# Hcyand/recommender_system

Measured on AMD Instinct MI355X. Metric: CTR forward samples/sec @ batch 4096, 26 sparse×1e7 vocab, dim 16; %HBM roofline, higher is better.
Workload: dtype f32

## Files before the change

### recommender_system_amd/csrc/capi.cpp

```cpp
#include <stdarg.h>
#include <stdio.h>

#include "rs_common.hpp"

namespace rs {
static thread_local char g_err[512] = "";

void set_error(const char* fmt, ...) {
  va_list ap;
  va_start(ap, fmt);
  vsnprintf(g_err, sizeof(g_err), fmt, ap);
  va_end(ap);
}

int launch_status(const char* what) {
  hipError_t e = hipGetLastError();
  if (e != hipSuccess) {
    set_error("%s: HIP launch failed: %s", what, hipGetErrorString(e));
    return RS_ERR_HIP;
  }
  return RS_OK;
}

static thread_local int g_opt[RS_OPT_COUNT] = {0, 1, 0, 0, 0, 0};
static const int g_opt_hi[RS_OPT_COUNT] = {5, 1, 3, 1, 1, 1};
int opt(int option) { return (option >= 0 && option < RS_OPT_COUNT) ? g_opt[option] : 0; }
}

extern "C" int rs_set_option(int option, int value) {
  if (option < 0 || option >= RS_OPT_COUNT || value < 0 || value > rs::g_opt_hi[option]) {
    rs::set_error("rs_set_option: unknown option %d or value %d out of range", option, value);
    return -1;
  }
  const int prev = rs::g_opt[option];
  rs::g_opt[option] = value;
  return prev;
}

extern "C" int rs_get_option(int option) {
  return (option >= 0 && option < RS_OPT_COUNT) ? rs::g_opt[option] : -1;
}

extern "C" const char* rs_version(void) { return "recommender_system_amd 0.1.0 (gfx950)"; }
extern "C" const char* rs_last_error_string(void) { return rs::g_err; }
```

### recommender_system_amd/csrc/deepfm.hip

```cpp
#include <stdlib.h>

#include <type_traits>

#include "embed_fm_body.hpp"
#include "rs_common.hpp"

namespace rs {

template <int KV, int KIND>
__global__ __launch_bounds__(16 * 64) void deepfm_fused(EmbedFmArgs a, MlpArgs t) {
  embed_fm_body<KV, 1, 16, KIND, true, 1>(a, &t, blockIdx.x);
}
template <int KV, int KIND>
__global__ __launch_bounds__(16 * 64) void deepfm_fused_ka(EmbedFmArgs a, MlpArgs t, FieldMeta m) {
  embed_fm_body<KV, 1, 16, KIND, true, 1, false, true>(a, &t, blockIdx.x, &m);
}

constexpr int WS_NL = 8;

__device__ __forceinline__ void lds_wait_ge(int* p, int v, int* err) {
  for (int spins = 0; __hip_atomic_load(p, __ATOMIC_ACQUIRE, __HIP_MEMORY_SCOPE_WORKGROUP) < v; ++spins) {
    if (spins > (1 << 22)) {
      if ((threadIdx.x & 63) == 0) flag_error(err, RS_FLAG_TIMEOUT);
      break;
    }
    __builtin_amdgcn_s_sleep(1);
  }
}
__device__ __forceinline__ void lds_signal(int* p) {
  if ((threadIdx.x & 63) == 0) __hip_atomic_fetch_add(p, 1, __ATOMIC_RELEASE, __HIP_MEMORY_SCOPE_WORKGROUP);
}

template <int KIND, int G, int GWA = 0, int GWB = 0>
__global__ __launch_bounds__(16 * 64) void deepfm_ws(EmbedFmArgs a, MlpArgs t, FieldMeta m) {
  typedef Ids<KIND> I;
  constexpr int NW = 16, F = G - 1, MF = (F + WS_NL - 1) / WS_NL;
  static_assert(F <= 32 && MF <= 4, "deepfm_ws: <= 32 fields");
  extern __shared__ float tsm[];
  __shared__ floatx4 lf_acc[WS_NL][64];
  __shared__ floatx4 lf_q[WS_NL][4];
  __shared__ float fmlog[16];
  __shared__ int cnt[4];
  const int lane = threadIdx.x & 63;
  const int w = __builtin_amdgcn_readfirstlane(threadIdx.x >> 6);
  const int s = lane & 15, kk = lane >> 4;
  const int64_t bt = (int64_t)blockIdx.x * 16 + s;
  const bool valid = bt < a.batch;
  const int64_t b = valid ? bt : a.batch - 1;
  const int RS = t.rs;
  float* par = tsm + 32 * RS + NW * 256;
  floatx4 ring[MLP_R];
  {
    const MlpArgs& a = t;
    MLP_STAMP(0);
  }
  if (threadIdx.x < 4) cnt[threadIdx.x] = 0;
  if (w < WS_NL) {
    const int l = w;
    const float w0v = a.w0[0];
    const int dw = l - (WS_NL - a.DB);
    const bool has_dense = dw >= 0;
    float dx = 0.f, drec = 0.f, dn = 0.f;
    if (has_dense) {
      const int e = 4 * dw + kk;
      dx = a.dense[b * a.dense_stride + (e < a.nd ? e : 0)];
      const float* rec = a.prep + (int64_t)dw * a.dense_rec;
      drec = rec[lane];
      dn = rec[64 + kk];
    }
    typename I::raw_t rid[MF];
    floatx4 bw[MF];
#pragma unroll
    for (int p = 0; p < MF; ++p) {
      const int c = l + WS_NL * p;
      bw[p] = floatx4{0.f, 0.f, 0.f, 0.f};
      if (c < F) {
        rid[p] = I::load(a.ids, b * a.id_stride + c);
        if (s <= a.kfm) bw[p] = *reinterpret_cast<const floatx4*>(a.prep + a.field_base + (int64_t)c * a.field_rec + lane * 4);
      }
    }
    floatx4 xs0[2];
    bool ok0[2];
#pragma unroll
    for (int q = 0; q < 2; ++q) {
      const int c = l + WS_NL * q;
      ok0[q] = false;
      if (q < MF && c < F) {
        int64_t id;
        ok0[q] = I::decode(rid[q], m.voc[c], id);
        xs0[q] = __builtin_nontemporal_load(reinterpret_cast<const floatx4*>(a.table + (m.off[c] + id) * 16) + kk);
      }
    }
    __syncthreads();
    floatx4 ac[4];
#pragma unroll
    for (int c = 0; c < 4; ++c) ac[c] = floatx4{0.f, 0.f, 0.f, 0.f};
    float qn = 0.f;
    if (has_dense) {
      const int e = 4 * dw + kk;
      const float x = e < a.nd ? dx : 0.f;
      ac[0] = mfma16x16x4(x, drec, ac[0]);
      qn = fmaf(x * x, dn, qn);
      tsm[s * RS + F * 16 + e] = x;
      lds_signal(&cnt[0]);
    }
    float nrm[MF][4];
#pragma unroll
    for (int p = 0; p < MF; ++p)
#pragma unroll
      for (int tp = 0; tp < 4; ++tp) nrm[p][tp] = row16_sum(s < a.kfm ? bw[p][tp] * bw[p][tp] : 0.f);
    bool bad = false;
#pragma unroll
    for (int burst = 0; burst < 2; ++burst) {
      floatx4 xs[2];
      bool ok[2];
#pragma unroll
      for (int q = 0; q < 2; ++q) {
        const int p = 2 * burst + q, c = l + WS_NL * p;
        if (burst == 0) {
          xs[q] = xs0[q];
          ok[q] = ok0[q];
          continue;
        }
        ok[q] = false;
        if (p < MF && c < F) {
          int64_t id;
          ok[q] = I::decode(rid[p], m.voc[c], id);
          xs[q] = __builtin_nontemporal_load(reinterpret_cast<const floatx4*>(a.table + (m.off[c] + id) * 16) + kk);
        }
      }
#pragma unroll
      for (int q = 0; q < 2; ++q) {
        const int p = 2 * burst + q, c = l + WS_NL * p;
        if (p < MF && c < F) {
          bad |= !ok[q];
          const floatx4 x = ok[q] ? xs[q] : floatx4{0.f, 0.f, 0.f, 0.f};
          *reinterpret_cast<floatx4*>(tsm + s * RS + c * 16 + 4 * kk) = x;
#pragma unroll
          for (int tp = 0; tp < 4; ++tp) {
            ac[tp] = mfma16x16x4(x[tp], bw[p][tp], ac[tp]);
            qn = fmaf(x[tp] * x[tp], nrm[p][tp], qn);
          }
        }
      }
#ifdef RS_DIAG_STAMPS
      if (!(burst == 1 && (a.ablate & 32)))
#endif
      lds_signal(&cnt[1 + burst]);
      {
        const MlpArgs& a = t;
        MLP_STAMP(2 + burst);
      }
    }
    if (__any(bad && valid) && lane == 0) flag_error(a.err);
    floatx4 acc;
#pragma unroll
    for (int i = 0; i < 4; ++i) acc[i] = (ac[0][i] + ac[1][i]) + (ac[2][i] + ac[3][i]);
    lf_acc[l][lane] = acc;
    qn += __shfl_xor(qn, 16);
    qn += __shfl_xor(qn, 32);
    if (lane < 16) reinterpret_cast<float*>(&lf_q[l][0])[lane] = qn;
    int old = 0;
    if (lane == 0) old = __hip_atomic_fetch_add(&cnt[3], 1, __ATOMIC_ACQ_REL, __HIP_MEMORY_SCOPE_WORKGROUP);
    old = __builtin_amdgcn_readfirstlane(old);
    if (old == WS_NL - 1) {
      floatx4 v = {0.f, 0.f, 0.f, 0.f};
#pragma unroll
      for (int ww = 0; ww < WS_NL; ++ww) {
        const floatx4 pv = lf_acc[ww][lane];
#pragma unroll
        for (int i = 0; i < 4; ++i) v[i] += pv[i];
      }
      const floatx4 q4 = lf_q[s < WS_NL ? s : 0][kk];
#pragma unroll
      for (int i = 0; i < 4; ++i) {
        float tt = s < a.kfm ? v[i] * v[i] : 0.f;
        if (s < WS_NL) tt -= q4[i];
        float ll = s == a.kfm ? v[i] : 0.f;
        tt = row16_sum(tt);
        ll = row16_sum(ll);
        const float fm = (ll + w0v) + 0.5f * tt;
        const int64_t bb = (int64_t)blockIdx.x * 16 + 4 * kk + i;
        if (s == 0) {
          fmlog[4 * kk + i] = fm;
          if (bb < a.batch && a.logit) a.logit[bb] = fm;
        }
      }
    }
  } else {
    const int c8 = w - WS_NL;
    const floatx4* W0 = reinterpret_cast<const floatx4*>(t.prep + t.off[0]) + lane + (int64_t)c8 * G * 64;
    const floatx4* W1 = W0 + (int64_t)WS_NL * G * 64;
    auto grp = [](int i) { return i == 0 ? G - 1 : i - 1; };
    floatx4 r0[3], r1[3];
#pragma unroll
    for (int u = 0; u < 3; ++u) {
      r0[u] = W0[(int64_t)grp(u) * 64];
      r1[u] = W1[(int64_t)grp(u) * 64];
    }
    __syncthreads();
    for (int i = threadIdx.x - WS_NL * 64; i < t.ptot; i += (NW - WS_NL) * 64) par[i] = t.prep[t.wtot + i];
    const int ecol0 = 16 * c8 + s, ecol1 = ecol0 + 16 * WS_NL;
    const float* pb = t.prep + t.wtot + t.poff[0];
    const float eb0 = pb[ecol0], eb1 = pb[ecol1], ea0 = pb[t.Np[0] + ecol0], ea1 = pb[t.Np[0] + ecol1];
    const float* ap = tsm + s * RS + 4 * kk;
    floatx4 acc0 = {0.f, 0.f, 0.f, 0.f}, acc1 = acc0, acc0b = acc0, acc1b = acc0;
    lds_wait_ge(&cnt[0], a.DB, a.err);
    auto step = [&](int i, auto U) {
      constexpr int u = decltype(U)::value;
      const floatx4 av = *reinterpret_cast<const floatx4*>(ap + 16 * grp(i));
      __builtin_amdgcn_sched_barrier(0);
#pragma unroll
      for (int j = 0; j < 4; j += 2) {
        acc0 = mfma16x16x4(av[j], r0[u][j], acc0);
        acc1 = mfma16x16x4(av[j], r1[u][j], acc1);
        acc0b = mfma16x16x4(av[j + 1], r0[u][j + 1], acc0b);
        acc1b = mfma16x16x4(av[j + 1], r1[u][j + 1], acc1b);
      }
      const int nx = i + 3 < G ? i + 3 : G - 1;
      r0[u] = W0[(int64_t)grp(nx) * 64];
      r1[u] = W1[(int64_t)grp(nx) * 64];
      __builtin_amdgcn_sched_barrier(0);
    };
    using U0 = std::integral_constant<int, 0>;
    using U1 = std::integral_constant<int, 1>;
    using U2 = std::integral_constant<int, 2>;
    auto wait_burst = [&](int which) {
      lds_wait_ge(&cnt[1 + which], WS_NL, a.err);
      const MlpArgs& a = t;
      MLP_STAMP(2 + which);
    };
    constexpr int B1 = 1 + 2 * WS_NL;
    if (t.unroll) {
#pragma unroll
      for (int i = 0; i < G; ++i) {
        if (i == 1) wait_burst(0);
        if (i == B1) wait_burst(1);
        if (i % 3 == 0) step(i, U0{});
        else if (i % 3 == 1) step(i, U1{});
        else step(i, U2{});
      }
    } else {
      static_assert((B1 - 2) % 3 == 0 && (G - 1 - B1) % 3 == 0, "deepfm_ws: group / ring phase");
      step(0, U0{});
      wait_burst(0);
      int i = 1;
#pragma unroll 1
      for (; i + 2 < B1; i += 3) {
        step(i, U1{});
        step(i + 1, U2{});
        step(i + 2, U0{});
      }
      step(i, U1{});
      wait_burst(1);
#pragma unroll 1
      for (i = B1; i + 2 < G; i += 3) {
        step(i, U2{});
        step(i + 1, U0{});
        step(i + 2, U1{});
      }
      step(i, U2{});
    }
#pragma unroll
    for (int i = 0; i < 4; ++i) {
      acc0[i] += acc0b[i];
      acc1[i] += acc1b[i];
    }
    float* out = tsm + 16 * RS;
    with_act(t.act[0], [&](auto A) {
#pragma unroll
      for (int r = 0; r < 4; ++r) {
        const int row = 4 * kk + r;
        out[row * RS + ecol0] = mlp_act_c<decltype(A)::value>(acc0[r] + eb0, ea0);
        out[row * RS + ecol1] = mlp_act_c<decltype(A)::value>(acc1[r] + eb1, ea1);
      }
    });
  }
  {
    const MlpArgs& a = t;
    MLP_STAMP(1);
  }
  if constexpr (GWA > 0) {
    if constexpr (GWA == 8 && GWB == 2) {
      mlp_tail_run<NW>(t, tsm, (int64_t)blockIdx.x * 16, fmlog);
    } else {
      floatx4 wr[GWA];
      mlp_tail_fetch<GWA>(t, 1, wr);
      mlp_tail_splitk<NW, GWA, GWB>(t, tsm, (int64_t)blockIdx.x * 16, wr, fmlog, 1);
    }
  } else {
    {
      const int T1 = t.Np[1] >> 4, G1 = t.Kp[1] >> 4;
      const int S1 = mlp_slices(T1, G1, NW);
      if (w < T1 * S1) {
        const MlpItem it = mlp_item(w, T1, G1, S1);
        mlp_ring_fill(ring, reinterpret_cast<const floatx4*>(t.prep + t.off[1]) + lane + (int64_t)it.t * G1 * 64,
                      it.g0, it.g1);
      }
    }
    mlp_tower_tile<NW>(t, tsm, (int64_t)blockIdx.x * 16, ring, fmlog, 1);
  }
}

template <int KIND, int G, int RD, int GWA = 0, int GWB = 0>
__global__ __launch_bounds__(16 * 64) void deepfm_all(EmbedFmArgs a, MlpArgs t, FieldMeta m) {
  typedef Ids<KIND> I;
  constexpr int NW = 16, F = G - 1;
  static_assert(F > 16 && F <= 32, "deepfm_all: 17..32 fields (two per wave at most)");
  static_assert(RD == 3 || RD == 4, "deepfm_all: weight ring 3 or 4 k-groups deep");
  extern __shared__ float tsm[];
  __shared__ floatx4 fm_acc[NW][64];
  __shared__ float fm_q[NW][16];
  __shared__ float fmlog[16];
  const int lane = threadIdx.x & 63;
  const int w = __builtin_amdgcn_readfirstlane(threadIdx.x >> 6);
  const int s = lane & 15, kk = lane >> 4;
  const int64_t bt = (int64_t)blockIdx.x * 16 + s;
  const bool valid = bt < a.batch;
  const int64_t b = valid ? bt : a.batch - 1;
  const int RS = t.rs;
  float* par = tsm + 32 * RS + NW * 256;
  {
    const MlpArgs& a = t;
    MLP_STAMP(0);
  }
  const int c0 = w, c1 = w + 16 < F ? w + 16 : w;
  const bool two = w + 16 < F;
  const typename I::raw_t rid0 = I::load(a.ids, b * a.id_stride + c0);
  const typename I::raw_t rid1 = I::load(a.ids, b * a.id_stride + c1);
  const int dw = w - (NW - 4);
  const bool has_dense = dw >= 0 && dw < a.DB;
  const int dwc = dw < 0 ? 0 : (dw < a.DB ? dw : 0);
  const int de = 4 * dwc + kk;
  const float dxv = a.dense[b * a.dense_stride + (de < a.nd ? de : 0)];
  int64_t id0, id1;
  const bool ok0 = I::decode(rid0, m.voc[c0], id0);
  const bool ok1 = I::decode(rid1, m.voc[c1], id1);
  const floatx4 x0 = __builtin_nontemporal_load(reinterpret_cast<const floatx4*>(a.table + (m.off[c0] + id0) * 16) + kk);
  const floatx4* x1p = reinterpret_cast<const floatx4*>(a.table + (m.off[c1] + id1) * 16) + kk;
  const floatx4* W0 = reinterpret_cast<const floatx4*>(t.prep + t.off[0]) + lane + (int64_t)w * G * 64;
  auto grp = [](int i) { return i == 0 ? G - 1 : i - 1; };
  floatx4 ring[RD];
#pragma unroll
  for (int u = 0; u < RD; ++u) ring[u] = W0[(int64_t)grp(u) * 64];
  const float* drec = a.prep + (int64_t)dwc * a.dense_rec;
  const float drv = drec[lane], dnv = drec[64 + kk];
  const floatx4 bw0 = *reinterpret_cast<const floatx4*>(a.prep + a.field_base + (int64_t)c0 * a.field_rec + lane * 4);
  const floatx4 bw1 = *reinterpret_cast<const floatx4*>(a.prep + a.field_base + (int64_t)c1 * a.field_rec + lane * 4);
  const float w0v = a.w0[0];
  const int npar = t.ptot;
  const int pi = threadIdx.x < npar ? threadIdx.x : 0;
  const float pv = t.prep[t.wtot + pi];
  bool bad = !ok0 || (two && !ok1);
  MacAcc<4> L0;
  const float* ap = tsm + s * RS + 4 * kk;
  floatx4 an = {0.f, 0.f, 0.f, 0.f};
  auto seg_start = [&](int i) { an = *reinterpret_cast<const floatx4*>(ap + 16 * grp(i)); };
  auto step = [&](int i, auto U) {
    constexpr int u = decltype(U)::value;
    const floatx4 av = an;
    if (i != 16 && i + 1 < G) an = *reinterpret_cast<const floatx4*>(ap + 16 * grp(i + 1));
    __builtin_amdgcn_sched_barrier(0);
    L0.mac4(av, ring[u]);
    if (i + RD < G) ring[u] = W0[(int64_t)grp(i + RD) * 64];
    __builtin_amdgcn_sched_barrier(0);
  };
  auto step_i = [&](int i) {
    switch (i % RD) {
      case 0: step(i, std::integral_constant<int, 0>{}); break;
      case 1: step(i, std::integral_constant<int, 1>{}); break;
      case 2: step(i, std::integral_constant<int, 2>{}); break;
      default: step(i, std::integral_constant<int, (RD > 3 ? 3 : 0)>{}); break;
    }
  };
  floatx4 fa = {0.f, 0.f, 0.f, 0.f};
  float qn = 0.f;
  if (dw >= 0) {
    const int e = 4 * dw + kk;
    const float x = e < a.nd ? dxv : 0.f;
    tsm[s * RS + F * 16 + e] = x;
    if (has_dense) {
      fa = mfma16x16x4(x, drv, fa);
      qn = fmaf(x * x, dnv, qn);
    }
  }
  float n0[4], n1[4];
#pragma unroll
  for (int tp = 0; tp < 4; ++tp) {
    n0[tp] = row16_sum(s < a.kfm ? bw0[tp] * bw0[tp] : 0.f);
    n1[tp] = row16_sum(s < a.kfm ? bw1[tp] * bw1[tp] : 0.f);
  }
  if (threadIdx.x < npar) par[pi] = pv;
  auto put_row = [&](int c, const floatx4& xr, bool ok, const floatx4& bw, const float (&nr)[4]) {
    const floatx4 x = ok ? xr : floatx4{0.f, 0.f, 0.f, 0.f};
    *reinterpret_cast<floatx4*>(tsm + s * RS + c * 16 + 4 * kk) = x;
#pragma unroll
    for (int tp = 0; tp < 4; ++tp) {
      fa = mfma16x16x4(x[tp], bw[tp], fa);
      qn = fmaf(x[tp] * x[tp], nr[tp], qn);
    }
  };
  put_row(c0, x0, ok0, bw0, n0);
  __syncthreads();
  {
    const MlpArgs& a = t;
    MLP_STAMP(2);
  }
  const floatx4 x1 = __builtin_nontemporal_load(x1p);
  __builtin_amdgcn_sched_barrier(0);
  seg_start(0);
#pragma unroll
  for (int i = 0; i <= 16; ++i) {
    step_i(i);
    if (i == 8) {
      if (two) put_row(c1, x1, ok1, bw1, n1);
      fm_acc[w][lane] = fa;
      qn += __shfl_xor(qn, 16);
      qn += __shfl_xor(qn, 32);
      if (lane < 16) fm_q[w][lane] = qn;
      if (__any(bad && valid) && lane == 0) flag_error(a.err);
    }
  }
  __syncthreads();
  {
    const MlpArgs& a = t;
    MLP_STAMP(3);
  }
  float fmv[NW];
  {
    const int ln = (w >> 2) * 16 + s, r = w & 3;
#pragma unroll
    for (int ww = 0; ww < NW; ++ww) fmv[ww] = fm_acc[ww][ln][r];
  }
  const float fq = fm_q[s][w];
  seg_start(17);
#pragma unroll
  for (int i = 17; i < G; ++i) step_i(i);
  const floatx4 acc0 = L0.sum();
  constexpr bool TAIL = GWA > 0;
  floatx4 wr[TAIL ? GWA : 1];
  floatx4 tring[MLP_R];
  if constexpr (TAIL) {
    mlp_tail_fetch<GWA>(t, 1, wr);
  } else {
    const int T1 = t.Np[1] >> 4, G1 = t.Kp[1] >> 4;
    const int S1 = mlp_slices(T1, G1, NW);
    if (w < T1 * S1) {
      const MlpItem it = mlp_item(w, T1, G1, S1);
      mlp_ring_fill(tring, reinterpret_cast<const floatx4*>(t.prep + t.off[1]) + lane + (int64_t)it.t * G1 * 64,
                    it.g0, it.g1);
    }
  }
  {
    float* out = tsm + 16 * RS;
    const int col = 16 * w + s;
    const float bc = par[t.poff[0] + col], ac = par[t.poff[0] + t.Np[0] + col];
    with_act(t.act[0], [&](auto A) {
#pragma unroll
      for (int r = 0; r < 4; ++r) out[(4 * kk + r) * RS + col] = mlp_act_c<decltype(A)::value>(acc0[r] + bc, ac);
    });
  }
  {
    float v = 0.f;
#pragma unroll
    for (int ww = 0; ww < NW; ++ww) v += fmv[ww];
    float tq = (s < a.kfm ? v * v : 0.f) - fq;
    float lin = s == a.kfm ? v : 0.f;
    tq = row16_sum(tq);
    lin = row16_sum(lin);
    const float fm = (lin + w0v) + 0.5f * tq;
    if (lane == 0) {
      fmlog[w] = fm;
      const int64_t bb = (int64_t)blockIdx.x * 16 + w;
      if (bb < a.batch && a.logit) a.logit[bb] = fm;
    }
  }
  {
    const MlpArgs& a = t;
    MLP_STAMP(1);
  }
  if constexpr (TAIL) {
    if constexpr (GWA == 8 && GWB == 2) mlp_tail_dispatch<NW>(t, tsm, (int64_t)blockIdx.x * 16, wr, fmlog, 1);
    else mlp_tail_splitk<NW, GWA, GWB>(t, tsm, (int64_t)blockIdx.x * 16, wr, fmlog, 1);
  }
  else mlp_tower_tile<NW>(t, tsm, (int64_t)blockIdx.x * 16, tring, fmlog, 1);
}

static bool deepfm_geom(int nd, int n_fields, int k, int kfm, int n_layers, const int* dims, FmGeom& fg,
                        MlpGeom& mg) {
  if (nd < 0 || n_fields < 1 || n_fields > 128 || kfm < 1 || (k != 8 && k != 16)) return false;
  fg = fm_geom(nd, n_fields, k, kfm);
  if (!fg.mfma || fg.NT != 1) return false;
  if (!mlp_geom(n_layers, dims, mg)) return false;
  return dims[0] == nd + n_fields * k && dims[n_layers] == 1 && mg.lds <= 120 * 1024;
}

static bool deepfm_ws_ok(const EmbedFmArgs& a, const MlpArgs& t, const FieldMeta* hm, int KV) {
  return hm && KV == 4 && a.F == 26 && a.nd >= 13 && a.nd <= 16 && a.DB == 4 && t.L >= 2 &&
         t.Np[0] == 256 && t.Kp[0] == 16 * (a.F + 1) && (t.Np[1] >> 4) >= WS_NL &&
         opt(RS_OPT_DEEPFM_KERNEL) == 0;
}

static bool deepfm_all_ok(const EmbedFmArgs& a, const MlpArgs& t, const FieldMeta* hm, int KV) {
  return hm && KV == 4 && a.F == 26 && a.nd >= 1 && a.nd <= 16 && a.DB <= 4 && t.L >= 2 && t.Np[0] == 256 &&
         t.Kp[0] == 16 * (a.F + 1) && t.ptot <= 1024 && opt(RS_OPT_DEEPFM_KERNEL) >= 2;
}

template <int KV, int KIND>
static void launch_deepfm(const EmbedFmArgs& a, const MlpArgs& t, size_t lds, hipStream_t st,
                          const FieldMeta* hm) {
  const unsigned grid = (unsigned)((a.batch + 15) / 16);
  if constexpr (KV == 4) {
    if (deepfm_all_ok(a, t, hm, KV)) {
      int gwa = 0, gwb = 0;
      const bool tail = mlp_tail_ok(t.Np, t.Kp, t.N, t.L, 1, gwa, gwb) && gwa == 8 && gwb == 2;
      const bool ring4 = opt(RS_OPT_DEEPFM_KERNEL) == 3;
      if (tail && ring4) launch_lds<deepfm_all<KIND, 27, 4, 8, 2>>(grid, 16 * 64, lds, st, a, t, *hm);
      else if (tail) launch_lds<deepfm_all<KIND, 27, 3, 8, 2>>(grid, 16 * 64, lds, st, a, t, *hm);
      else launch_lds<deepfm_all<KIND, 27, 3>>(grid, 16 * 64, lds, st, a, t, *hm);
      return;
    }
    if (deepfm_ws_ok(a, t, hm, KV)) {
      int gwa = 0, gwb = 0;
      if (mlp_tail_ok(t.Np, t.Kp, t.N, t.L, 1, gwa, gwb) && gwa == 8 && gwb == 2)
        launch_lds<deepfm_ws<KIND, 27, 8, 2>>(grid, 16 * 64, lds, st, a, t, *hm);
      else launch_lds<deepfm_ws<KIND, 27>>(grid, 16 * 64, lds, st, a, t, *hm);
      return;
    }
  }
  if (hm && a.F <= 32 && a.DB <= 16) launch_lds<deepfm_fused_ka<KV, KIND>>(grid, 16 * 64, lds, st, a, t, *hm);
  else launch_lds<deepfm_fused<KV, KIND>>(grid, 16 * 64, lds, st, a, t);
}

}

using namespace rs;

extern "C" int rs_deepfm_fused_ok(int nd, int n_fields, int k, int kfm, int n_layers, const int* dims) {
  FmGeom fg;
  MlpGeom mg;
  return dims && deepfm_geom(nd, n_fields, k, kfm, n_layers, dims, fg, mg) ? 1 : 0;
}

static int deepfm_run(const void* ids, int id_kind, int64_t id_stride, const float* dense, int64_t dense_stride,
                      int nd, const float* table, const int64_t* field_offsets, const int64_t* field_vocab,
                      int n_fields, int k, const float* fm_prepared, const float* w0, int kfm, int n_layers,
                      const int* dims, const int* acts, const float* mlp_prepared, float c0, float c1, float* out,
                      float* fm_logit, int64_t batch, int* err_flag, rs_stream_t stream, const FieldMeta* hm) {
  if (batch == 0) return RS_OK;
  FmGeom fg;
  MlpGeom mg;
  RS_REQUIRE(dims && acts, "rs_deepfm_fwd: null dims/acts");
  RS_REQUIRE(deepfm_geom(nd, n_fields, k, kfm, n_layers, dims, fg, mg),
             "rs_deepfm_fwd: unsupported shape (see rs_deepfm_fused_ok)");
  RS_REQUIRE(batch >= 0 && ids && table && field_offsets && field_vocab && fm_prepared && w0 && mlp_prepared && out,
             "rs_deepfm_fwd: null pointer");
  RS_REQUIRE(nd == 0 || dense, "rs_deepfm_fwd: dense is null");
  RS_REQUIRE(id_kind >= RS_ID_I32 && id_kind <= RS_ID_F32, "rs_deepfm_fwd: bad id_kind");
  RS_REQUIRE((uintptr_t)table % 16 == 0, "rs_deepfm_fwd: table must be 16-B aligned");
  MlpArgs t{};
  RS_REQUIRE(mlp_fill_args(mg, acts, mlp_prepared, t), "rs_deepfm_fwd: bad activation");
  t.y = out;
  t.ys = 1;
  t.head = 1;
  t.c0 = c0;
  t.c1 = c1;
  t.M = batch;
  t.dbg = mlp_diag_dbg();
  EmbedFmArgs a = fm_args(ids, id_stride, dense, dense_stride, nd, table, field_offsets, field_vocab, n_fields, k,
                          fm_prepared, w0, kfm, fm_logit, nullptr, batch, err_flag);
  set_geom(a, fg);
#ifdef RS_DIAG_STAMPS
  a.ablate = getenv("RS_ABLATE") ? atoi(getenv("RS_ABLATE")) : 0;
#endif
  hipStream_t st = as_stream(stream);
  with_id_kind(id_kind, [&](auto K) {
    constexpr int KIND = decltype(K)::value;
    if (fg.KV == 2) launch_deepfm<2, KIND>(a, t, mg.lds, st, hm);
    else launch_deepfm<4, KIND>(a, t, mg.lds, st, hm);
  });
  return launch_status("rs_deepfm_fwd");
}

extern "C" int rs_deepfm_fwd(const void* ids, int id_kind, int64_t id_stride, const float* dense,
                             int64_t dense_stride, int nd, const float* table, const int64_t* field_offsets,
                             const int64_t* field_vocab, int n_fields, int k, const float* fm_prepared,
                             const float* w0, int kfm, int n_layers, const int* dims, const int* acts,
                             const float* mlp_prepared, float c0, float c1, float* out, float* fm_logit,
                             int64_t batch, int* err_flag, rs_stream_t stream) {
  return deepfm_run(ids, id_kind, id_stride, dense, dense_stride, nd, table, field_offsets, field_vocab, n_fields, k,
                    fm_prepared, w0, kfm, n_layers, dims, acts, mlp_prepared, c0, c1, out, fm_logit, batch, err_flag,
                    stream, nullptr);
}

extern "C" int rs_deepfm_fwd_hm(const void* ids, int id_kind, int64_t id_stride, const float* dense,
                                int64_t dense_stride, int nd, const float* table, const int64_t* field_offsets,
                                const int64_t* field_vocab, const int64_t* field_offsets_host,
                                const int64_t* field_vocab_host, int n_fields, int k, const float* fm_prepared,
                                const float* w0, int kfm, int n_layers, const int* dims, const int* acts,
                                const float* mlp_prepared, float c0, float c1, float* out, float* fm_logit,
                                int64_t batch, int* err_flag, rs_stream_t stream) {
  RS_REQUIRE(batch == 0 || (field_offsets_host && field_vocab_host), "rs_deepfm_fwd_hm: host metadata missing");
  const bool use = n_fields <= 32 && batch > 0;
  const FieldMeta m = field_meta(field_offsets_host, field_vocab_host, use ? n_fields : 0);
  return deepfm_run(ids, id_kind, id_stride, dense, dense_stride, nd, table, field_offsets, field_vocab, n_fields, k,
                    fm_prepared, w0, kfm, n_layers, dims, acts, mlp_prepared, c0, c1, out, fm_logit, batch, err_flag,
                    stream, use ? &m : nullptr);
}
```

### recommender_system_amd/csrc/embed_fm.hip

```cpp
#include <stdlib.h>

#include <type_traits>

#include "embed_fm_body.hpp"
#include "rs_common.hpp"

namespace rs {

__device__ __forceinline__ float fm_bval(const float* w1, const float* v, int d, int kfm, int e, int colg) {
  if (e >= d) return 0.f;
  if (colg < kfm) return v[(int64_t)e * kfm + colg];
  if (colg == kfm) return w1[e];
  return 0.f;
}

__device__ __forceinline__ float fm_rownorm(const float* v, int d, int kfm, int e) {
  if (e >= d) return 0.f;
  float n = 0.f;
  for (int f = 0; f < kfm; ++f) {
    const float t = v[(int64_t)e * kfm + f];
    n = fmaf(t, t, n);
  }
  return n;
}

__global__ void fm_prepare_mfma(const float* __restrict__ w1, const float* __restrict__ v, int nd, int F,
                                int k, int kfm, int KV, int NT, int DB, int64_t dense_rec,
                                int64_t field_rec, int64_t field_base, int64_t size,
                                float* __restrict__ out) {
  const int d = nd + F * k;
  for (int64_t idx = (int64_t)blockIdx.x * blockDim.x + threadIdx.x; idx < size;
       idx += (int64_t)gridDim.x * blockDim.x) {
    float val;
    if (idx < field_base) {
      const int t = (int)(idx / dense_rec);
      const int r = (int)(idx % dense_rec);
      if (r < NT * 64) {
        const int nt = r / 64, lane = r % 64;
        const int e = 4 * t + (lane >> 4);
        val = (e < nd) ? fm_bval(w1, v, d, kfm, e, nt * 16 + (lane & 15)) : 0.f;
      } else {
        const int e = 4 * t + (r - NT * 64);
        val = (e < nd) ? fm_rownorm(v, d, kfm, e) : 0.f;
      }
    } else {
      const int64_t j = idx - field_base;
      const int c = (int)(j / field_rec);
      const int r = (int)(j % field_rec);
      if (r < NT * 64 * KV) {
        const int nt = r / (64 * KV), rem = r % (64 * KV);
        const int lane = rem / KV, tp = rem % KV;
        const int e = nd + c * k + KV * (lane >> 4) + tp;
        val = fm_bval(w1, v, d, kfm, e, nt * 16 + (lane & 15));
      } else {
        const int r2 = r - NT * 64 * KV;
        const int e = nd + c * k + KV * (r2 / KV) + (r2 % KV);
        val = fm_rownorm(v, d, kfm, e);
      }
    }
    out[idx] = val;
  }
}

__global__ void fm_prepare_generic(const float* __restrict__ w1, const float* __restrict__ v, int d, int kfm,
                                   float* __restrict__ out) {
  const int64_t n = (int64_t)d * (kfm + 2);
  for (int64_t idx = (int64_t)blockIdx.x * blockDim.x + threadIdx.x; idx < n;
       idx += (int64_t)gridDim.x * blockDim.x) {
    float val;
    if (idx < d) val = w1[idx];
    else if (idx < (int64_t)d * (kfm + 1)) val = v[idx - d];
    else val = fm_rownorm(v, d, kfm, (int)(idx - (int64_t)d * (kfm + 1)));
    out[idx] = val;
  }
}

template <int KV, int NT, int NW, int KIND, int MC, bool PF = false>
__global__ __launch_bounds__(NW * 64) void embed_fm_mfma(EmbedFmArgs a) {
  embed_fm_body<KV, NT, NW, KIND, false, MC, PF>(a, nullptr, blockIdx.x);
}

template <int KV, int NT, int NW, int KIND, bool PF, int FC = 0, int KFMC = 0, int NDC = -1, bool ID1 = false>
__global__ __launch_bounds__(NW * 64) void embed_fm_mfma_ka(EmbedFmArgs a, FieldMeta m) {
  embed_fm_body<KV, NT, NW, KIND, false, 1, PF, true, FC, KFMC, NDC, false, ID1>(a, nullptr, blockIdx.x, &m);
}

template <int KV, int NT, int FC, int KFMC, int NDC>
static bool ct_geom_matches(const EmbedFmArgs& a) {
  constexpr FmGeom G = fm_geom(NDC, FC, 4 * KV, KFMC);
  return G.mfma && G.KV == KV && G.NT == NT && a.F == FC && a.kfm == KFMC && a.nd == NDC && a.k == 4 * KV &&
         a.DB == G.DB && a.dense_rec == G.dense_rec && a.field_rec == G.field_rec && a.field_base == G.field_base;
}

static int headline_spec(const EmbedFmArgs& a) {
  if (a.F != 26 || a.kfm != 10 || a.nd != 13 || a.k != 16) return 0;
  return ct_geom_matches<4, 1, 26, 10, 13>(a) ? 1 : -1;
}

template <int KV, int NT, int NW, int KIND, bool PF, int FC = 0, int KFMC = 0, int NDC = -1, bool ID1 = false>
__global__ __launch_bounds__(NW * 64) void embed_fm_mfma_kp(const float* prep, const void* ids, int64_t id_stride,
                                                            int64_t batch, const float* dense, int64_t dense_stride,
                                                            const float* table, EmbedFmCold c, FieldMeta m) {
  const EmbedFmArgs a = hot_cold_args<KV, NT, FC, KFMC, NDC>(prep, ids, id_stride, batch, dense, dense_stride, table, c);
  embed_fm_body<KV, NT, NW, KIND, false, 1, PF, true, FC, KFMC, NDC, true, ID1>(a, nullptr, blockIdx.x, &m);
}

struct StreamArgs {
  int tpb, S;
  int64_t ids_bstride_bytes, dense_bstride, logit_bstride, last_batch;
};
template <int KV, int NT, int KIND, int FC = 0, int KFMC = 0, int NDC = -1>
__global__ __launch_bounds__(16 * 64) void embed_fm_stream_ka(EmbedFmArgs a, FieldMeta m, StreamArgs sa) {
  const int s = blockIdx.x / sa.tpb, tile = blockIdx.x - s * sa.tpb;
  EmbedFmArgs b = a;
  b.ids = static_cast<const char*>(a.ids) + s * sa.ids_bstride_bytes;
  b.dense = a.dense + s * sa.dense_bstride;
  b.logit = a.logit + s * sa.logit_bstride;
  if (s == sa.S - 1) b.batch = sa.last_batch;
  if ((int64_t)tile * 16 >= b.batch) return;
  embed_fm_body<KV, NT, 16, KIND, false, 1, true, true, FC, KFMC, NDC>(b, nullptr, tile, &m);
}
template <int KV, int NT, int KIND, int FC = 0, int KFMC = 0, int NDC = -1>
__global__ __launch_bounds__(16 * 64) void embed_fm_stream_kp(const float* prep, const void* ids, int64_t id_stride,
                                                              int64_t batch, const float* dense, int64_t dense_stride,
                                                              const float* table, EmbedFmCold c, FieldMeta m,
                                                              StreamArgs sa) {
  const int s = blockIdx.x / sa.tpb, tile = blockIdx.x - s * sa.tpb;
  EmbedFmArgs b = hot_cold_args<KV, NT, FC, KFMC, NDC>(prep, ids, id_stride, batch, dense, dense_stride, table, c);
  b.ids = static_cast<const char*>(ids) + s * sa.ids_bstride_bytes;
  b.dense = dense + s * sa.dense_bstride;
  b.logit = c.logit + s * sa.logit_bstride;
  if (s == sa.S - 1) b.batch = sa.last_batch;
  if ((int64_t)tile * 16 >= b.batch) return;
  embed_fm_body<KV, NT, 16, KIND, false, 1, true, true, FC, KFMC, NDC, true>(b, nullptr, tile, &m);
}

__device__ __forceinline__ float block_sum(float v, float* red) {
#pragma unroll
  for (int o = 32; o > 0; o >>= 1) v += __shfl_xor(v, o);
  const int lane = threadIdx.x & 63, w = threadIdx.x >> 6;
  __syncthreads();
  if (lane == 0) red[w] = v;
  __syncthreads();
  float t = 0.f;
  for (int i = 0; i < (int)(blockDim.x >> 6); ++i) t += red[i];
  return t;
}

template <int KIND>
__global__ __launch_bounds__(256) void embed_fm_generic(EmbedFmArgs a) {
  typedef Ids<KIND == 3 ? 0 : KIND> I;
  __shared__ int64_t rows[1024];
  __shared__ float red[4];
  const int64_t b = blockIdx.x;
  const int d = a.nd + a.F * a.k;
  const float* w1 = a.prep;
  const float* v = a.prep + d;
  const float* nsq = a.prep + (int64_t)d * (a.kfm + 1);
  for (int c = threadIdx.x; c < a.F; c += blockDim.x) {
    int64_t row = b * a.F + c;
    if constexpr (KIND != 3) {
      int64_t id;
      if (I::decode(I::load(a.ids, b * a.id_stride + c), a.vocab[c], id)) row = a.offs[c] + id;
      else { row = -1; flag_error(a.err); }
    }
    rows[c] = row;
  }
  __syncthreads();
  auto xval = [&](int e) -> float {
    if (e < a.nd) return a.dense[b * a.dense_stride + e];
    const int c = (e - a.nd) / a.k, j = (e - a.nd) % a.k;
    const int64_t r = rows[c];
    return r >= 0 ? a.table[r * a.k + j] : 0.f;
  };
  float lin = 0.f, q = 0.f;
  for (int e = threadIdx.x; e < d; e += blockDim.x) {
    const float x = xval(e);
    lin = fmaf(x, w1[e], lin);
    q = fmaf(x * x, nsq[e], q);
    if (a.x_out) a.x_out[b * d + e] = x;
  }
  lin = block_sum(lin, red);
  q = block_sum(q, red);
  float ss = 0.f;
  for (int f = 0; f < a.kfm; ++f) {
    float p = 0.f;
    for (int e = threadIdx.x; e < d; e += blockDim.x) p = fmaf(xval(e), v[(int64_t)e * a.kfm + f], p);
    p = block_sum(p, red);
    ss = fmaf(p, p, ss);
  }
  if (threadIdx.x == 0) a.logit[b] = (lin + a.w0[0]) + 0.5f * (ss - q);
}

constexpr bool kKernargPreloadDefault = true;
static bool kernarg_preload() {
  const int v = opt(RS_OPT_EMBED_FM_KERNEL);
  return v == 5 || (v != 4 && kKernargPreloadDefault);
}

template <int KV, int NT, int KIND>
static void launch_embed_fm3(const EmbedFmArgs& a, hipStream_t st, const FieldMeta* hm) {
  const int grid = (int)((a.batch + 15) / 16);
  if constexpr (KIND != 3) {
    if (hm && a.F <= 32 && grid <= 512 && a.DB <= 16 && !a.x_out) {
      const bool pl = kernarg_preload();
      const EmbedFmCold c = cold_args(a);
      if constexpr (KV == 4 && NT == 1 && KIND != 2) {
        if (headline_spec(a) == 1) {
          if (pl)
            embed_fm_mfma_kp<KV, NT, 16, KIND, true, 26, 10, 13, true><<<grid, 16 * 64, 0, st>>>(
                a.prep, a.ids, a.id_stride, a.batch, a.dense, a.dense_stride, a.table, c, *hm);
          else embed_fm_mfma_ka<KV, NT, 16, KIND, true, 26, 10, 13, true><<<grid, 16 * 64, 0, st>>>(a, *hm);
          return;
        }
      }
      constexpr bool ID1 = KIND != 2 && KV * NT <= 8;
      if (pl)
        embed_fm_mfma_kp<KV, NT, 16, KIND, true, 0, 0, -1, ID1><<<grid, 16 * 64, 0, st>>>(
            a.prep, a.ids, a.id_stride, a.batch, a.dense, a.dense_stride, a.table, c, *hm);
      else embed_fm_mfma_ka<KV, NT, 16, KIND, true, 0, 0, -1, ID1><<<grid, 16 * 64, 0, st>>>(a, *hm);
      return;
    }
  }
  if (a.F <= 32 && grid > 1024) embed_fm_mfma<KV, NT, 4, KIND, 1, true><<<grid, 4 * 64, 0, st>>>(a);
  else if (a.F <= 32 && grid > 512) embed_fm_mfma<KV, NT, 8, KIND, 1, true><<<grid, 8 * 64, 0, st>>>(a);
  else if (a.F <= 32) embed_fm_mfma<KV, NT, 16, KIND, 1><<<grid, 16 * 64, 0, st>>>(a);
  else embed_fm_mfma<KV, NT, 16, KIND, 0><<<grid, 16 * 64, 0, st>>>(a);
}

template <int KIND>
static void launch_embed_fm_k(const EmbedFmArgs& a, int KV, int NT, hipStream_t st,
                              const FieldMeta* hm = nullptr) {
  with_kv(KV, [&](auto kv) {
    constexpr int V = decltype(kv)::value;
    if (NT == 1) launch_embed_fm3<V, 1, KIND>(a, st, hm);
    else launch_embed_fm3<V, 2, KIND>(a, st, hm);
  });
}

static int run_embed_fm(EmbedFmArgs a, const FmGeom& g, int kind, hipStream_t st, const char* what,
                        const FieldMeta* hm = nullptr) {
  if (a.batch == 0) return RS_OK;
  if (g.mfma) {
    set_geom(a, g);
    if (a.F == 0) {
// ... 326 lines not shown
```

### recommender_system_amd/csrc/embed_fm_body.hpp

```cpp
#pragma once
#include "embed_fm.hpp"
#include "mlp_tower.hpp"

namespace rs {

#ifdef RS_DIAG_STAMPS
#define RS_STAMP(i)                                                                          \
  do {                                                                                       \
    __builtin_amdgcn_sched_barrier(0);                                                       \
    if (a.dbg && lane == 0)                                                                  \
      a.dbg[((int64_t)blockIdx.x * NW + w) * 16 + (i)] = __builtin_amdgcn_s_memrealtime();  \
    __builtin_amdgcn_sched_barrier(0);                                                       \
  } while (0)
#define RS_USE(x) asm volatile("" ::"v"(x))
#else
#define RS_STAMP(i) \
  do {              \
  } while (0)
#define RS_USE(x) \
  do {            \
  } while (0)
#endif

template <int KV, int NT, int NW, int KIND, bool TW, int MC = 0, bool PF = false, bool KA = false, int FC = 0,
// ... 364 lines not shown
      } else if (a.x_out && valid && e < and_) {
        a.x_out[b * d + e] = x;
      }
    }
  }
  floatx4 acc[NT];
#pragma unroll
  for (int nt = 0; nt < NT; ++nt)
#pragma unroll
    for (int i = 0; i < 4; ++i) acc[nt][i] = (ac[nt][0][i] + ac[nt][1][i]) + (ac[nt][2][i] + ac[nt][3][i]);
  RS_USE(acc[0][0]);
  RS_STAMP(3);
  if (__any(bad && valid) && lane == 0) flag_error(a.err);

#ifdef RS_DIAG_STAMPS
  if (a.ablate & 4) {
    if (w == 0 && kk == 0 && b < a.batch) a.logit[b] = acc[0][0] + acc[0][1] + qn;
    return;
  }
#endif
#pragma unroll
  for (int nt = 0; nt < NT; ++nt)
#pragma unroll
    for (int r = 0; r < 4; ++r) {
      const int smp = kk * 4 + r, col = nt * 16 + s;
      cs[WIDE ? (smp * NC + col) * CW + w : (w * 16 + smp) * (NC + 1) + col] = acc[nt][r];
    }
  __builtin_amdgcn_sched_barrier(0);
  const auto h = __builtin_amdgcn_permlane16_swap(__float_as_uint(qn), __float_as_uint(qn), false, false);
  qn = __uint_as_float(h[0]) + __uint_as_float(h[1]);
  const auto f = __builtin_amdgcn_permlane32_swap(__float_as_uint(qn), __float_as_uint(qn), false, false);
  qn = __uint_as_float(f[0]) + __uint_as_float(f[1]);
  if (lane < 16) qs[w][lane] = qn;
  __syncthreads();
  RS_STAMP(7);
  if (threadIdx.x < 16 * NC) {
    const int smp = threadIdx.x / NC, col = threadIdx.x % NC;
    float v = 0.f;
    if constexpr (WIDE) {
      const floatx4* pw = reinterpret_cast<const floatx4*>(cs + (smp * NC + col) * CW);
      floatx4 pv[NW / 4];
#pragma unroll
      for (int g = 0; g < NW / 4; ++g) pv[g] = pw[g];
#pragma unroll
      for (int ww = 0; ww < NW; ++ww) v += pv[ww / 4][ww % 4];
    } else {
#pragma unroll
      for (int ww = 0; ww < NW; ++ww) v += cs[(ww * 16 + smp) * (NC + 1) + col];
    }
    float t = col < akfm ? v * v : 0.f;
    if (col < NW) t -= qs[col][smp];
    float lin = col == akfm ? v : 0.f;
    t = row16_sum(t);
    lin = row16_sum(lin);
    if constexpr (NT == 2) {
      t += __shfl_xor(t, 16);
      lin += __shfl_xor(lin, 16);
    }
    const int64_t bb = (int64_t)tile * 16 + smp;
    if constexpr (OWNER) {
      float q = col < NW ? qs[col][smp] : 0.f;
      q = row16_sum(q);
      if constexpr (NT == 2) q += __shfl_xor(q, 16);
      if (bb < a.batch) {
        float* rec = a.logit + bb * a.pstride;
        if (col <= akfm) rec[col] = v;
        if (col == 0) rec[akfm + 1] = q;
        else if (akfm + 1 + col < a.pw) rec[akfm + 1 + col] = 0.f;
      }
      return;
    }
    const float fm = (lin + w0v) + 0.5f * t;
    if (col == 0 && bb < a.batch && a.logit) a.logit[bb] = fm;
    if constexpr (TW) {
      if (col == 0) fmlog[smp] = fm;
    }
  }
  RS_STAMP(4);
  if constexpr (TW) {
    {
      const MlpArgs& a = *tw;
      MLP_STAMP(1);
    }
    mlp_tower_tile<NW>(*tw, tsm, (int64_t)tile * 16, ring, fmlog);
  }
}

struct EmbedFmCold {
  float* logit;
  const float* w0;
  int* err;
  int F, k, nd, kfm;
  const int64_t* offs;
  const int64_t* vocab;
  float* x_out;
  int DB;
  int64_t dense_rec, field_rec, field_base;
  int64_t owner_rows;
  int pw;
  int64_t pstride;
  unsigned long long* dbg;
  int ablate;
};

static inline EmbedFmCold cold_args(const EmbedFmArgs& a) {
  return EmbedFmCold{a.logit, a.w0,        a.err,       a.F,          a.k,          a.nd, a.kfm,     a.offs, a.vocab,
                     a.x_out, a.DB,        a.dense_rec, a.field_rec,  a.field_base, a.owner_rows,    a.pw,   a.pstride,
                     a.dbg,   a.ablate};
}

template <int KV, int NT, int FC, int KFMC, int NDC>
__device__ __forceinline__ EmbedFmArgs hot_cold_args(const float* prep, const void* ids, int64_t id_stride,
                                                     int64_t batch, const float* dense, int64_t dense_stride,
                                                     const float* table, const EmbedFmCold& c) {
  EmbedFmArgs a;
  a.ids = ids;
  a.id_stride = id_stride;
  a.dense = dense;
  a.dense_stride = dense_stride;
  a.nd = c.nd;
  a.table = table;
  a.offs = c.offs;
  a.vocab = c.vocab;
  a.F = c.F;
  a.k = c.k;
  a.prep = prep;
  a.w0 = c.w0;
  a.kfm = c.kfm;
  a.logit = c.logit;
  a.x_out = c.x_out;
  a.batch = batch;
  a.err = c.err;
  if constexpr (FC > 0) {
    constexpr FmGeom G = fm_geom(NDC, FC, 4 * KV, KFMC);
    static_assert(G.mfma && G.KV == KV && G.NT == NT, "specialised shape: not this instantiation's geometry");
    a.DB = G.DB;
    a.dense_rec = G.dense_rec;
    a.field_rec = G.field_rec;
    a.field_base = G.field_base;
  } else {
    a.DB = c.DB;
    a.dense_rec = c.dense_rec;
    a.field_rec = c.field_rec;
    a.field_base = c.field_base;
  }
  a.owner_rows = c.owner_rows;
  a.pw = c.pw;
  a.pstride = c.pstride;
  a.dbg = c.dbg;
  a.ablate = c.ablate;
  return a;
}

}
```

Measured before the change: 791.7 million.

## Add specialised front end to warp-specialised DeepFM kernel with early id/weight loads

Adds a front-end path to the deepfm_ws kernel that issues id, FM weight and dense loads before the MLP weight staging. It also hoists per-field offsets and vocab sizes into scalar registers and, for integer ids, loads one id per lane and redistributes them with permlane swaps. A compile-time specialisation for the 26-field, kfm=10, nd=13 shape bakes geometry constants into the kernel. The aim is to cut load latency and index arithmetic on the embedding gather critical path, at the cost of more template instantiations, register pressure, and a 32-bit batch index restriction. The old path stays available through option value 4.

After: 791.6 million (median of 4 runs). About the same (-0.0%).

```diff
diff --git a/recommender_system_amd/csrc/capi.cpp b/recommender_system_amd/csrc/capi.cpp
--- a/recommender_system_amd/csrc/capi.cpp
+++ b/recommender_system_amd/csrc/capi.cpp
@@ -23,7 +23,7 @@
 }
 
 static thread_local int g_opt[RS_OPT_COUNT] = {0, 1, 0, 0, 0, 0};
-static const int g_opt_hi[RS_OPT_COUNT] = {5, 1, 3, 1, 1, 1};
+static const int g_opt_hi[RS_OPT_COUNT] = {5, 1, 4, 1, 1, 1};
 int opt(int option) { return (option >= 0 && option < RS_OPT_COUNT) ? g_opt[option] : 0; }
 }
 
diff --git a/recommender_system_amd/csrc/deepfm.hip b/recommender_system_amd/csrc/deepfm.hip
--- a/recommender_system_amd/csrc/deepfm.hip
+++ b/recommender_system_amd/csrc/deepfm.hip
@@ -31,8 +31,9 @@
   if ((threadIdx.x & 63) == 0) __hip_atomic_fetch_add(p, 1, __ATOMIC_RELEASE, __HIP_MEMORY_SCOPE_WORKGROUP);
 }
 
-template <int KIND, int G, int GWA = 0, int GWB = 0>
-__global__ __launch_bounds__(16 * 64) void deepfm_ws(EmbedFmArgs a, MlpArgs t, FieldMeta m) {
+template <int KIND, int G, int GWA, int GWB, bool FE, int KFMC, int NDC, bool ID1>
+__device__ __forceinline__ void deepfm_ws_body(const EmbedFmArgs& a, const MlpArgs& t, const FieldMeta& m) {
+  static_assert(!ID1 || (FE && KIND < 2), "ID1: integer ids, the new front end");
   typedef Ids<KIND> I;
   constexpr int NW = 16, F = G - 1, MF = (F + WS_NL - 1) / WS_NL;
   static_assert(F <= 32 && MF <= 4, "deepfm_ws: <= 32 fields");
@@ -46,9 +47,50 @@
   const int s = lane & 15, kk = lane >> 4;
   const int64_t bt = (int64_t)blockIdx.x * 16 + s;
   const bool valid = bt < a.batch;
-  const int64_t b = valid ? bt : a.batch - 1;
+  const int64_t b = FE ? (int64_t)(uint32_t)(valid ? (int)bt : (int)a.batch - 1) : (valid ? bt : a.batch - 1);
+  const int akfm = KFMC > 0 ? KFMC : a.kfm;
+  const int and_ = NDC >= 0 ? NDC : a.nd;
+  const int dw = w - (WS_NL - a.DB);
+  const bool has_dense = dw >= 0;
+  float dx = 0.f, drec = 0.f, dn = 0.f;
+  typename I::raw_t rid[MF];
+  floatx4 bw[MF];
+  auto has = [&](int p) { return p < MF && (WS_NL * p + WS_NL - 1 < F || w + WS_NL * p < F); };
+  if constexpr (FE) {
+    static_assert(!ID1 || MF == 4, "ID1: one id per k-slot");
+    if (w < WS_NL) {
+      const int l = w;
+      auto load_b = [&]() {
+#pragma unroll
+        for (int p = 0; p < MF; ++p) {
+          bw[p] = floatx4{0.f, 0.f, 0.f, 0.f};
+          if (has(p))
+            bw[p] = *reinterpret_cast<const floatx4*>(a.prep + a.field_base + (int64_t)(l + WS_NL * p) * a.field_rec + lane * 4);
+        }
+      };
+      auto load_ids = [&]() {
+        if constexpr (ID1) {
+          const int c = l + WS_NL * kk;
+          rid[0] = I::load(a.ids, b * a.id_stride + (c < F ? c : l));
+        } else {
+#pragma unroll
+          for (int p = 0; p < MF; ++p)
+            if (has(p)) rid[p] = I::load(a.ids, b * a.id_stride + (l + WS_NL * p));
+        }
+      };
+      load_b();
+      load_ids();
+      if (has_dense) {
+        const int e = 4 * dw + kk;
+        dx = a.dense[b * a.dense_stride + (e < and_ ? e : 0)];
+        const float* rec = a.prep + (int64_t)dw * a.dense_rec;
+        drec = rec[lane];
+        dn = rec[64 + kk];
+      }
+    }
+    __builtin_amdgcn_sched_barrier(0);
+  }
   const int RS = t.rs;
-  float* par = tsm + 32 * RS + NW * 256;
   floatx4 ring[MLP_R];
   {
     const MlpArgs& a = t;
@@ -57,38 +99,90 @@
   if (threadIdx.x < 4) cnt[threadIdx.x] = 0;
   if (w < WS_NL) {
     const int l = w;
-    const float w0v = a.w0[0];
-    const int dw = l - (WS_NL - a.DB);
-    const bool has_dense = dw >= 0;
-    float dx = 0.f, drec = 0.f, dn = 0.f;
-    if (has_dense) {
-      const int e = 4 * dw + kk;
-      dx = a.dense[b * a.dense_stride + (e < a.nd ? e : 0)];
-      const float* rec = a.prep + (int64_t)dw * a.dense_rec;
-      drec = rec[lane];
-      dn = rec[64 + kk];
-    }
-    typename I::raw_t rid[MF];
-    floatx4 bw[MF];
-#pragma unroll
-    for (int p = 0; p < MF; ++p) {
-      const int c = l + WS_NL * p;
-      bw[p] = floatx4{0.f, 0.f, 0.f, 0.f};
-      if (c < F) {
-        rid[p] = I::load(a.ids, b * a.id_stride + c);
-        if (s <= a.kfm) bw[p] = *reinterpret_cast<const floatx4*>(a.prep + a.field_base + (int64_t)c * a.field_rec + lane * 4);
-      }
-    }
+    if constexpr (FE) __builtin_assume(l >= 0 && l < WS_NL);
+    float w0v = 0.f;
+    int64_t moff[MF], mvoc[MF];
     floatx4 xs0[2];
     bool ok0[2];
-#pragma unroll
-    for (int q = 0; q < 2; ++q) {
-      const int c = l + WS_NL * q;
-      ok0[q] = false;
-      if (q < MF && c < F) {
-        int64_t id;
-        ok0[q] = I::decode(rid[q], m.voc[c], id);
-        xs0[q] = __builtin_nontemporal_load(reinterpret_cast<const floatx4*>(a.table + (m.off[c] + id) * 16) + kk);
+    if constexpr (FE) {
+      w0v = a.w0[0];
+#pragma unroll
+      for (int p = 0; p < MF; ++p) {
+        moff[p] = mvoc[p] = 0;
+        if (has(p)) {
+          moff[p] = m.off[l + WS_NL * p];
+          mvoc[p] = m.voc[l + WS_NL * p];
+        }
+      }
+#pragma unroll
+      for (int p = 0; p < MF; ++p) asm volatile("" ::"s"(moff[p]), "s"(mvoc[p]));
+      unsigned hlo[2] = {0, 0}, hhi[2] = {0, 0};
+      if constexpr (ID1) {
+        const uint64_t r = (uint64_t)(int64_t)rid[0];
+        const auto h = __builtin_amdgcn_permlane32_swap((unsigned)r, (unsigned)r, false, false);
+        hlo[0] = h[0];
+        hlo[1] = h[1];
+        const auto g = __builtin_amdgcn_permlane16_swap(hlo[0], hlo[0], false, false);
+        if constexpr (sizeof(typename I::raw_t) == 4) {
+          rid[0] = (typename I::raw_t)(int32_t)g[0];
+          rid[1] = (typename I::raw_t)(int32_t)g[1];
+        } else {
+          const auto hh = __builtin_amdgcn_permlane32_swap((unsigned)(r >> 32), (unsigned)(r >> 32), false, false);
+          hhi[0] = hh[0];
+          hhi[1] = hh[1];
+          const auto gh = __builtin_amdgcn_permlane16_swap(hhi[0], hhi[0], false, false);
+          rid[0] = (typename I::raw_t)((uint64_t)gh[0] << 32 | g[0]);
+          rid[1] = (typename I::raw_t)((uint64_t)gh[1] << 32 | g[1]);
+        }
+      }
+#pragma unroll
+      for (int q = 0; q < 2; ++q) {
+        ok0[q] = false;
+        if (has(q)) {
+          int64_t id;
+          ok0[q] = I::decode(rid[q], mvoc[q], id);
+          xs0[q] = __builtin_nontemporal_load(reinterpret_cast<const floatx4*>(a.table + (moff[q] + id) * 16) + kk);
+        }
+      }
+      if constexpr (ID1) {
+        __builtin_amdgcn_sched_barrier(0);
+        const auto g = __builtin_amdgcn_permlane16_swap(hlo[1], hlo[1], false, false);
+        if constexpr (sizeof(typename I::raw_t) == 4) {
+          rid[2] = (typename I::raw_t)(int32_t)g[0];
+          rid[3] = (typename I::raw_t)(int32_t)g[1];
+        } else {
+          const auto gh = __builtin_amdgcn_permlane16_swap(hhi[1], hhi[1], false, false);
+          rid[2] = (typename I::raw_t)((uint64_t)gh[0] << 32 | g[0]);
+          rid[3] = (typename I::raw_t)((uint64_t)gh[1] << 32 | g[1]);
+        }
+      }
+    } else {
+      w0v = a.w0[0];
+      if (has_dense) {
+        const int e = 4 * dw + kk;
+        dx = a.dense[b * a.dense_stride + (e < a.nd ? e : 0)];
+        const float* rec = a.prep + (int64_t)dw * a.dense_rec;
+        drec = rec[lane];
+        dn = rec[64 + kk];
+      }
+#pragma unroll
+      for (int p = 0; p < MF; ++p) {
+        const int c = l + WS_NL * p;
+        bw[p] = floatx4{0.f, 0.f, 0.f, 0.f};
+        if (c < F) {
+          rid[p] = I::load(a.ids, b * a.id_stride + c);
+          if (s <= a.kfm) bw[p] = *reinterpret_cast<const floatx4*>(a.prep + a.field_base + (int64_t)c * a.field_rec + lane * 4);
+        }
+      }
+#pragma unroll
+      for (int q = 0; q < 2; ++q) {
+        const int c = l + WS_NL * q;
+        ok0[q] = false;
+        if (q < MF && c < F) {
+          int64_t id;
+          ok0[q] = I::decode(rid[q], m.voc[c], id);
+          xs0[q] = __builtin_nontemporal_load(reinterpret_cast<const floatx4*>(a.table + (m.off[c] + id) * 16) + kk);
+        }
       }
     }
     __syncthreads();
@@ -98,7 +192,7 @@
     float qn = 0.f;
     if (has_dense) {
       const int e = 4 * dw + kk;
-      const float x = e < a.nd ? dx : 0.f;
+      const float x = e < and_ ? dx : 0.f;
       ac[0] = mfma16x16x4(x, drec, ac[0]);
       qn = fmaf(x * x, dn, qn);
       tsm[s * RS + F * 16 + e] = x;
@@ -108,7 +202,7 @@
 #pragma unroll
     for (int p = 0; p < MF; ++p)
 #pragma unroll
-      for (int tp = 0; tp < 4; ++tp) nrm[p][tp] = row16_sum(s < a.kfm ? bw[p][tp] * bw[p][tp] : 0.f);
+      for (int tp = 0; tp < 4; ++tp) nrm[p][tp] = row16_sum(s < akfm ? bw[p][tp] * bw[p][tp] : 0.f);
     bool bad = false;
 #pragma unroll
     for (int burst = 0; burst < 2; ++burst) {
@@ -125,8 +219,8 @@
         ok[q] = false;
         if (p < MF && c < F) {
           int64_t id;
-          ok[q] = I::decode(rid[p], m.voc[c], id);
-          xs[q] = __builtin_nontemporal_load(reinterpret_cast<const floatx4*>(a.table + (m.off[c] + id) * 16) + kk);
+          ok[q] = I::decode(rid[p], FE ? mvoc[p] : m.voc[c], id);
+          xs[q] = __builtin_nontemporal_load(reinterpret_cast<const floatx4*>(a.table + ((FE ? moff[p] : m.off[c]) + id) * 16) + kk);
         }
       }
 #pragma unroll
@@ -174,9 +268,9 @@
       const floatx4 q4 = lf_q[s < WS_NL ? s : 0][kk];
 #pragma unroll
       for (int i = 0; i < 4; ++i) {
-        float tt = s < a.kfm ? v[i] * v[i] : 0.f;
+        float tt = s < akfm ? v[i] * v[i] : 0.f;
         if (s < WS_NL) tt -= q4[i];
-        float ll = s == a.kfm ? v[i] : 0.f;
+        float ll = s == akfm ? v[i] : 0.f;
         tt = row16_sum(tt);
         ll = row16_sum(ll);
         const float fm = (ll + w0v) + 0.5f * tt;
@@ -189,6 +283,7 @@
     }
   } else {
     const int c8 = w - WS_NL;
+    float* par = tsm + 32 * RS + NW * 256;
     const floatx4* W0 = reinterpret_cast<const floatx4*>(t.prep + t.off[0]) + lane + (int64_t)c8 * G * 64;
     const floatx4* W1 = W0 + (int64_t)WS_NL * G * 64;
     auto grp = [](int i) { return i == 0 ? G - 1 : i - 1; };
@@ -300,6 +395,19 @@
     }
     mlp_tower_tile<NW>(t, tsm, (int64_t)blockIdx.x * 16, ring, fmlog, 1);
   }
+}
+
+template <int KIND, int G, int GWA = 0, int GWB = 0, bool FE = false, int KFMC = 0, int NDC = -1, bool ID1 = false>
+__global__ __launch_bounds__(16 * 64) void deepfm_ws(EmbedFmArgs a, MlpArgs t, FieldMeta m) {
+  if constexpr (KFMC > 0) {
+    constexpr FmGeom GG = fm_geom(NDC, G - 1, 16, KFMC);
+    static_assert(GG.mfma && GG.KV == 4 && GG.NT == 1, "specialised shape: not this kernel's geometry");
+    a.DB = GG.DB;
+    a.dense_rec = GG.dense_rec;
+    a.field_rec = GG.field_rec;
+    a.field_base = GG.field_base;
+  }
+  deepfm_ws_body<KIND, G, GWA, GWB, FE, KFMC, NDC, ID1>(a, t, m);
 }
 
 template <int KIND, int G, int RD, int GWA = 0, int GWB = 0>
@@ -498,12 +606,26 @@
 static bool deepfm_ws_ok(const EmbedFmArgs& a, const MlpArgs& t, const FieldMeta* hm, int KV) {
   return hm && KV == 4 && a.F == 26 && a.nd >= 13 && a.nd <= 16 && a.DB == 4 && t.L >= 2 &&
          t.Np[0] == 256 && t.Kp[0] == 16 * (a.F + 1) && (t.Np[1] >> 4) >= WS_NL &&
-         opt(RS_OPT_DEEPFM_KERNEL) == 0;
+         (opt(RS_OPT_DEEPFM_KERNEL) == 0 || opt(RS_OPT_DEEPFM_KERNEL) == 4);
+}
+
+static bool deepfm_ws_front_end(const EmbedFmArgs& a) {
+  return opt(RS_OPT_DEEPFM_KERNEL) == 0 && a.batch <= INT32_MAX;
+}
+template <int KIND, int GWA, int GWB>
+static void launch_deepfm_ws(unsigned grid, size_t lds, hipStream_t st, const EmbedFmArgs& a, const MlpArgs& t,
+                             const FieldMeta& m) {
+  constexpr bool ID1 = KIND < 2;
+  if (!deepfm_ws_front_end(a)) launch_lds<deepfm_ws<KIND, 27, GWA, GWB>>(grid, 16 * 64, lds, st, a, t, m);
+  else if (a.kfm == 10 && a.nd == 13 && ct_geom_matches<4, 1, 26, 10, 13>(a))
+    launch_lds<deepfm_ws<KIND, 27, GWA, GWB, true, 10, 13, ID1>>(grid, 16 * 64, lds, st, a, t, m);
+  else launch_lds<deepfm_ws<KIND, 27, GWA, GWB, true, 0, -1, ID1>>(grid, 16 * 64, lds, st, a, t, m);
 }
 
 static bool deepfm_all_ok(const EmbedFmArgs& a, const MlpArgs& t, const FieldMeta* hm, int KV) {
   return hm && KV == 4 && a.F == 26 && a.nd >= 1 && a.nd <= 16 && a.DB <= 4 && t.L >= 2 && t.Np[0] == 256 &&
-         t.Kp[0] == 16 * (a.F + 1) && t.ptot <= 1024 && opt(RS_OPT_DEEPFM_KERNEL) >= 2;
+         t.Kp[0] == 16 * (a.F + 1) && t.ptot <= 1024 &&
+         (opt(RS_OPT_DEEPFM_KERNEL) == 2 || opt(RS_OPT_DEEPFM_KERNEL) == 3);
 }
 
 template <int KV, int KIND>
@@ -523,8 +645,8 @@
     if (deepfm_ws_ok(a, t, hm, KV)) {
       int gwa = 0, gwb = 0;
       if (mlp_tail_ok(t.Np, t.Kp, t.N, t.L, 1, gwa, gwb) && gwa == 8 && gwb == 2)
-        launch_lds<deepfm_ws<KIND, 27, 8, 2>>(grid, 16 * 64, lds, st, a, t, *hm);
-      else launch_lds<deepfm_ws<KIND, 27>>(grid, 16 * 64, lds, st, a, t, *hm);
+        launch_deepfm_ws<KIND, 8, 2>(grid, lds, st, a, t, *hm);
+      else launch_deepfm_ws<KIND, 0, 0>(grid, lds, st, a, t, *hm);
       return;
     }
   }
diff --git a/recommender_system_amd/csrc/embed_fm.hip b/recommender_system_amd/csrc/embed_fm.hip
--- a/recommender_system_amd/csrc/embed_fm.hip
+++ b/recommender_system_amd/csrc/embed_fm.hip
@@ -85,12 +85,6 @@
   embed_fm_body<KV, NT, NW, KIND, false, 1, PF, true, FC, KFMC, NDC, false, ID1>(a, nullptr, blockIdx.x, &m);
 }
 
-template <int KV, int NT, int FC, int KFMC, int NDC>
-static bool ct_geom_matches(const EmbedFmArgs& a) {
-  constexpr FmGeom G = fm_geom(NDC, FC, 4 * KV, KFMC);
-  return G.mfma && G.KV == KV && G.NT == NT && a.F == FC && a.kfm == KFMC && a.nd == NDC && a.k == 4 * KV &&
-         a.DB == G.DB && a.dense_rec == G.dense_rec && a.field_rec == G.field_rec && a.field_base == G.field_base;
-}
 
 static int headline_spec(const EmbedFmArgs& a) {
   if (a.F != 26 || a.kfm != 10 || a.nd != 13 || a.k != 16) return 0;
diff --git a/recommender_system_amd/csrc/embed_fm_body.hpp b/recommender_system_amd/csrc/embed_fm_body.hpp
--- a/recommender_system_amd/csrc/embed_fm_body.hpp
+++ b/recommender_system_amd/csrc/embed_fm_body.hpp
@@ -540,4 +540,11 @@
   return a;
 }
 
+template <int KV, int NT, int FC, int KFMC, int NDC>
+static inline bool ct_geom_matches(const EmbedFmArgs& a) {
+  constexpr FmGeom G = fm_geom(NDC, FC, 4 * KV, KFMC);
+  return G.mfma && G.KV == KV && G.NT == NT && a.F == FC && a.kfm == KFMC && a.nd == NDC && a.k == 4 * KV &&
+         a.DB == G.DB && a.dense_rec == G.dense_rec && a.field_rec == G.field_rec && a.field_base == G.field_base;
 }
+
+}
```
